# saltoricristiano/lidog

Hardware: AMD Instinct MI355X
Metric: LiDAR scans/sec, MinkUNet34+BEV training step @120k pts (higher is better)
Workload: dtype f32

## Files before the change

### include/lidog_amd.h

```cpp
#ifndef LIDOG_AMD_H
#define LIDOG_AMD_H

#include <stdint.h>

#ifdef __cplusplus
extern "C" {
#endif

const char *lidog_last_error(void);
int lidog_abi_version(void);


int64_t lidog_hash_capacity(int64_t n);

int lidog_coords_insert(const int32_t *coords, int64_t n, uint64_t *keys, int32_t *vals, int64_t cap,
                        int32_t *first_row, int64_t *n_unique_dev, int32_t *err_flag, void *stream);
int lidog_coords_insert_info(const int32_t *coords, int64_t n, uint64_t *keys, int32_t *vals, int64_t cap,
                             int32_t *first_row, int64_t *info, int32_t *err_flag, void *stream);

int lidog_coords_compact(const int32_t *first_row, int64_t n, const uint64_t *keys, int32_t *vals, int64_t cap,
                         const int32_t *coords, int32_t *unique_rows, int32_t *inverse, int32_t *scan_ws,
                         void *stream);

int lidog_coords_stride(const int32_t *coords_in, int64_t n_in, int32_t new_stride, uint64_t *keys,
// ... 121 lines not shown
                       const int32_t *pixel, int64_t n, int32_t C, int32_t B, int32_t H, int32_t W, int32_t pk,
                       int32_t ps, int32_t pp, int32_t Ho, int32_t Wo, float *gfeats , void *stream);

int lidog_conv2d_fwd(const float *x, const float *w, const float *bias, int32_t B, int32_t Cin, int32_t H,
                     int32_t W, int32_t Cout, int32_t ksize, int32_t stride, int32_t pad, float *y, void *stream);
int lidog_conv2d_dgrad(const float *gy, const float *w, int32_t B, int32_t Cin, int32_t H, int32_t W,
                       int32_t Cout, int32_t ksize, int32_t stride, int32_t pad, float *gx, float *ws,
                       void *stream);
int lidog_conv2d_wgrad(const float *x, const float *gy, int32_t B, int32_t Cin, int32_t H, int32_t W,
                       int32_t Cout, int32_t ksize, int32_t stride, int32_t pad, float *gw, float *gbias,
                       float *ws, int64_t ws_floats, void *stream);

int64_t lidog_conv2d_support_ws(int32_t B, int32_t Cin, int32_t H, int32_t W);
int lidog_conv2d_support(const int32_t *support, int32_t B, int32_t Cin, int32_t H, int32_t W, int32_t *act,
                         void *stream);
int lidog_conv2d_fwd_sparse(const float *x, const float *w, const int32_t *act, int32_t B, int32_t Cin, int32_t H,
                            int32_t W, int32_t Cout, float *y, float *ws, void *stream);
int lidog_conv2d_dgrad_sparse(const float *gy, const float *w, const int32_t *act, int32_t B, int32_t Cin, int32_t H,
                              int32_t W, int32_t Cout, float *gx, float *ws, void *stream);
int lidog_conv2d_support_work(const int32_t *act, int32_t B, int32_t Cin, int32_t H, int32_t W, int32_t Cout,
                              double *out, void *stream);
int64_t lidog_conv2d_wgrad_sparse_ws(int32_t B, int32_t Cin, int32_t H, int32_t W, int32_t Cout);
int lidog_conv2d_wgrad_sparse(const float *x, const float *gy, const int32_t *act, int32_t B, int32_t Cin, int32_t H,
                              int32_t W, int32_t Cout, float *gw, float *ws, int64_t ws_floats, void *stream);

int64_t lidog_dice_ws(int32_t C);
int lidog_dice_fwd(const float *logits, const int64_t *target, int64_t n, int32_t C, int64_t ignore_label,
                   int32_t has_ignore, float eps, int32_t soft, int32_t powerize, int32_t use_tmask, float offset,
                   double *ws, float *loss, float *coef, void *stream);
int lidog_dice_bwd(const float *logits, const int64_t *target, int64_t n, int32_t C, int64_t ignore_label,
// ... 243 lines not shown
```

### lidog_amd/_lib.py

```python
import ctypes
import os

import torch

_HERE = os.path.dirname(os.path.abspath(__file__))
SO_PATH = os.environ.get("LIDOG_SO") or os.path.join(_HERE, "_C", "liblidog_amd.so")

_i32, _i64, _p, _f, _d = ctypes.c_int32, ctypes.c_int64, ctypes.c_void_p, ctypes.c_float, ctypes.c_double

SIGNATURES = {
    "lidog_abi_version": [],
    "lidog_hash_capacity": [_i64],
    "lidog_coords_insert": [_p, _i64, _p, _p, _i64, _p, _p, _p, _p],
    "lidog_coords_insert_info": [_p, _i64, _p, _p, _i64, _p, _p, _p, _p],
    "lidog_coords_compact": [_p, _i64, _p, _p, _i64, _p, _p, _p, _p, _p],
    "lidog_coords_stride": [_p, _i64, _i32, _p, _p, _i64, _p, _p, _p, _p, _p, _p],
    "lidog_kernel_map": [_p, _i64, _p, _p, _i64, _p, _i32, _p, _p],
    "lidog_bitmap_words": [_i32, _i32, _i32, _i32, _i64],
    "lidog_bitmap_set": [_p, _i64, _i32, _i32, _i32, _i32, _i32, _i32, _i32, _i32, _p, _p, _p],
    "lidog_kernel_map_bits": [_p, _i64, _p, _p, _i64, _p, _i32, _p, _i32, _i32, _i32, _i32, _i32, _i32, _i32, _i32, _p, _p],
    "lidog_kernel_map_pairs": [_p, _i64, _i64, _i32, _p, _p, _p, _p, _p, _p, _p],
    "lidog_sconv_gemm_units": [_i32, _i32],
    "lidog_sconv_gemm": [_p, _p, _p, _p, _p, _p, _p, _i32, _i32, _i32, _p, _p, _i64, _p],
    "lidog_sconv_gemm_addend": [_p, _p, _p, _p, _p, _p, _i32, _i32, _i32, _p, _p, _p, _p],
# ... 46 lines not shown
    "lidog_colsum_ws": [_i32],
    "lidog_bn_eval_invstd": [_p, _f, _i32, _p, _p],
    "lidog_cat2": [_p, _i32, _p, _i32, _i64, _p, _p],
    "lidog_split2": [_p, _i32, _i32, _i64, _p, _p, _p],
    "lidog_relu_fwd": [_p, _i64, _p, _p],
    "lidog_relu_bwd": [_p, _p, _i64, _p, _p],
    "lidog_add": [_p, _p, _i64, _p, _p],
    "lidog_bev_winner": [_p, _i64, _p, _p, _i32, _i32, _i32, _i32, _p, _p, _p],
    "lidog_bev_pool_fwd": [_p, _i32, _p, _p, _i64, _i32, _i32, _i32, _i32, _i32, _i32, _i32, _i32, _p, _p, _p, _p],
    "lidog_bev_pool_bwd": [_p, _p, _p, _p, _i64, _i32, _i32, _i32, _i32, _i32, _i32, _i32, _i32, _i32, _p, _p],
    "lidog_conv2d_fwd": [_p, _p, _p, _i32, _i32, _i32, _i32, _i32, _i32, _i32, _i32, _p, _p],
    "lidog_conv2d_dgrad": [_p, _p, _i32, _i32, _i32, _i32, _i32, _i32, _i32, _i32, _p, _p, _p],
    "lidog_conv2d_wgrad": [_p, _p, _i32, _i32, _i32, _i32, _i32, _i32, _i32, _i32, _p, _p, _p, _i64, _p],
    "lidog_conv2d_support_ws": [_i32, _i32, _i32, _i32],
    "lidog_conv2d_support": [_p, _i32, _i32, _i32, _i32, _p, _p],
    "lidog_conv2d_fwd_sparse": [_p, _p, _p, _i32, _i32, _i32, _i32, _i32, _p, _p, _p],
    "lidog_conv2d_dgrad_sparse": [_p, _p, _p, _i32, _i32, _i32, _i32, _i32, _p, _p, _p],
    "lidog_conv2d_wgrad_sparse_ws": [_i32, _i32, _i32, _i32, _i32],
    "lidog_conv2d_wgrad_sparse": [_p, _p, _p, _i32, _i32, _i32, _i32, _i32, _p, _p, _i64, _p],
    "lidog_voxel_floor": [_p, _i64, _f, _f, _f, _i32, _p, _p],
    "lidog_label_vote": [_p, _p, _p, _i64, _i64, _i32, _p, _p],
    "lidog_bev_label_raster": [_p, _p, _i64, _p, _p, _p, _i32, _i32, _i32, _i32, _p, _p, _p, _p],
    "lidog_dice_ws": [_i32],
    "lidog_dice_fwd": [_p, _p, _i64, _i32, _i64, _i32, _f, _i32, _i32, _i32, _f, _p, _p, _p, _p],
    "lidog_dice_bwd": [_p, _p, _i64, _i32, _i64, _i32, _f, _i32, _i32, _p, _p, _p, _p],
    "lidog_dice_kitti_fwd": [_p, _p, _i64, _i32, _i64, _i32, _f, _i32, _i32, _f, _p, _p, _p, _p],
    "lidog_dice_kitti_bwd": [_p, _p, _i64, _i32, _i64, _i32, _f, _i32, _p, _p, _p, _p],
    "lidog_ce_ws": [_i32],
    "lidog_ce_fwd": [_p, _p, _i64, _i32, _i64, _i32, _p, _i32, _d, _d, _p, _p, _p, _p],
    "lidog_ce_bwd": [_p, _p, _i64, _i32, _i64, _i32, _p, _p, _p, _p, _p],
# ... 160 lines not shown
```

### lidog_amd/bev.py

```python
import os

import numpy as np
import torch
import torch.nn as nn

from . import me as ME
from ._lib import call, ptr

_LUTS = {}
SPARSE_CONV1 = os.environ.get("LIDOG_CONV1_SPARSE", "1") != "0"


def bev_image_size(bound, voxel=0.05):
    return int(np.float32((bound - (-bound)) / voxel))


def pixel_luts(bound, voxel=0.05):
    key = (float(bound), float(voxel))
    if key not in _LUTS:
        H = bev_image_size(bound, voxel)
        lo, hi = -int(H * 0.6), int(H * 0.6)
        c = np.arange(lo, hi, dtype=np.int32)
        v = c.astype(np.float32) * np.float32(voxel)
        inb = (np.float32(-bound) < v) & (v < np.float32(bound))
# ... 111 lines not shown
        return {"launches": len(self.records), "total_ms": ms, "executed_flops": flops}


HEAD_TIMER = None


def _timed(work):
    import contextlib
    t = HEAD_TIMER
    return HeadTimer._Span(t, work) if (t is not None and t.enabled) else contextlib.nullcontext()


class _Conv2dFn(torch.autograd.Function):

    @staticmethod
    def forward(ctx, x, w, bias, ksize, stride, pad, support):
        x, w = x.contiguous(), w.contiguous()
        B, Cin, H, W = x.shape
        Cout = w.shape[0]
        Ho, Wo = (H + 2 * pad - ksize) // stride + 1, (W + 2 * pad - ksize) // stride + 1
        y = torch.empty((B, Cout, Ho, Wo), dtype=torch.float32, device=x.device)
        act = None
        if support is not None and (ksize, stride, pad) == (3, 2, 1) and bias is None and Cin <= 128 \
                and Cout % 128 == 0:
            n_act = ME._lib.load().lidog_conv2d_support_ws(B, Cin, H, W)
            if tuple(support.shape) == tuple(x.shape):
                act = torch.empty(n_act, dtype=torch.int32, device=x.device)
                call("lidog_conv2d_support", ptr(support), B, Cin, H, W, ptr(act))
            elif support.dim() == 1 and support.numel() == n_act:
                act = support
                call("lidog_conv2d_support", None, B, Cin, H, W, ptr(act))
        dense = 2.0 * B * Ho * Wo * Cout * Cin * ksize * ksize
        if act is not None:
            ws = torch.empty(9 * Cin * Cout, dtype=torch.float32, device=x.device)
            with _timed((act, (B, Cin, H, W, Cout), 0)):
                call("lidog_conv2d_fwd_sparse", ptr(x), ptr(w), ptr(act), B, Cin, H, W, Cout, ptr(y), ptr(ws))
        elif ksize == 3:
            with _timed(dense):
                call("lidog_conv2d_fwd", ptr(x), ptr(w), ptr(bias), B, Cin, H, W, Cout, ksize, stride, pad, ptr(y))
        else:
            call("lidog_conv2d_fwd", ptr(x), ptr(w), ptr(bias), B, Cin, H, W, Cout, ksize, stride, pad, ptr(y))
        ctx.save_for_backward(x, w, act)
        ctx.cfg = (ksize, stride, pad, bias is not None)
        ctx.params = (w, bias)
        return y

    @staticmethod
    def backward(ctx, gy):
        x, w, act = ctx.saved_tensors
        ksize, stride, pad, has_bias = ctx.cfg
        gy = gy.contiguous()
        B, Cin, H, W = x.shape
        Cout = w.shape[0]
        gx = gw = gb = None
        lane_on = ME._WgradLane.active()
        behind = lane_on and ME._WgradLane.mode == 2

        def queue_wgrad():
            gw = ME._grad_out(ctx.params[0], w.shape)
            gb = ME._grad_out(ctx.params[1], (Cout,)) if has_bias else None
            if act is not None:
                n_ws = ME._lib.load().lidog_conv2d_wgrad_sparse_ws(B, Cin, H, W, Cout)
            else:
                n_ws = 32 * w.numel() if ksize == 3 else 4 * B * (w.numel() + Cout)

            def wgrad(gw, gb):
                ws = torch.empty(max(n_ws, 1), dtype=torch.float32, device=x.device)
                if act is not None:
                    with _timed((act, (B, Cin, H, W, Cout), 2)):
# ... 19 lines not shown
        if ctx.needs_input_grad[1] and not behind:
            gw, gb = queue_wgrad()
        if ctx.needs_input_grad[0]:
            gx = torch.empty_like(x)
            ws = torch.empty(9 * Cin * Cout, dtype=torch.float32, device=x.device) if ksize == 3 else None
            if act is not None:
                with _timed((act, (B, Cin, H, W, Cout), 1)):
                    call("lidog_conv2d_dgrad_sparse", ptr(gy), ptr(w), ptr(act), B, Cin, H, W, Cout, ptr(gx), ptr(ws))
            elif ksize == 3:
                with _timed(2.0 * gy.shape[0] * gy.shape[2] * gy.shape[3] * Cout * Cin * 9):
                    call("lidog_conv2d_dgrad", ptr(gy), ptr(w), B, Cin, H, W, Cout, ksize, stride, pad, ptr(gx), ptr(ws))
            else:
                call("lidog_conv2d_dgrad", ptr(gy), ptr(w), B, Cin, H, W, Cout, ksize, stride, pad, ptr(gx), ptr(ws))
        if ctx.needs_input_grad[1] and gw is None:
            gw, gb = queue_wgrad()
        return gx, gw, gb, None, None, None, None


def conv2d(x, conv, support=None):
    k, s, p = conv.kernel_size[0], conv.stride[0], conv.padding[0]
    return _Conv2dFn.apply(x, conv.weight, conv.bias, k, s, p, support)


class Encoder2D(nn.Module):

    def __init__(self, input_size, n_classes=7, binary_seg=False):
        super().__init__()
        if binary_seg:
            raise NotImplementedError("binary_seg is off in every LiDOG config")
        dbl = nn.Module()
        dbl.double_conv = nn.Sequential(
            nn.Conv2d(input_size, 256, kernel_size=3, padding=1, stride=2, bias=False), nn.BatchNorm2d(256),
            nn.ReLU(inplace=True),
            nn.Conv2d(256, 256, kernel_size=3, padding=1, stride=2, bias=False), nn.BatchNorm2d(256),
            nn.ReLU(inplace=True))
        down = nn.Module()
# ... 15 lines not shown
```

### lidog_amd/csrc/conv2d.hip

```cpp
#include "common.h"
#include "clock_stamp.h"

#include "conv2d.h"

#define WG_LD 129
__global__ __launch_bounds__(256) void k_conv_wgrad(IgParams p) {
    __shared__ float As[C2_KB * WG_LD];
    __shared__ float Bs[C2_KB * WG_LD];
    const int tid = threadIdx.x, lane = tid & 63, wave = tid >> 6;
    const int i0 = blockIdx.y * IG_T, j0 = blockIdx.x * IG_T;
    const int HoWo = p.Ho * p.Wo;
    const int k_begin = blockIdx.z * p.k_chunk;
    const int k_end = k_begin + p.k_chunk < p.Kd ? k_begin + p.k_chunk : p.Kd;
    const int kk = tid & 31, rg = tid >> 5;

    int cpk[16];
    unsigned a_mask = 0;
#pragma unroll
    for (int r = 0; r < 16; ++r) {
        int j = j0 + rg + 8 * r;
        cpk[r] = -1;
        int ci = j / 9;
        if (j < p.Nj) cpk[r] = wgrad_col(p, ci, j - ci * 9);
        a_mask |= (unsigned)(i0 + rg + 8 * r < p.Mi) << r;
// ... 164 lines not shown
void lidog_launch_repack_dgrad_all(const float *W, int Cin, int Cout, float *Wd, hipStream_t st) {
    const int64_t total = 9 * (int64_t)Cin * Cout;
    k_repack_dgrad_all<<<(unsigned)cdiv64(total, 256), 256, 0, st>>>(W, Cin, Cout, Wd);
}

__global__ __launch_bounds__(256) void k_sum_splits(const float *__restrict__ partial, int64_t n, int splits,
                                                    int64_t stride, float *__restrict__ out) {
    int64_t i = (int64_t)blockIdx.x * 256 + threadIdx.x;
    if (i >= n) return;
    float acc = partial[i];
    for (int s = 1; s < splits; ++s) acc += partial[(size_t)s * stride + i];
    out[i] = acc;
}

#define PW_MAXCO 8
__global__ __launch_bounds__(256) void k_pw_fwd(const float *__restrict__ X, const float *__restrict__ W,
                                                const float *__restrict__ bias, int Cin, int Cout, int64_t HW,
                                                int64_t total, float *__restrict__ Y) {
    int64_t e = (int64_t)blockIdx.x * 256 + threadIdx.x;
    if (e >= total) return;
    int64_t b = e / HW, pix = e - b * HW;
    float acc[PW_MAXCO];
#pragma unroll
    for (int co = 0; co < PW_MAXCO; ++co) acc[co] = 0.f;
    const float *x = X + (size_t)b * Cin * HW + pix;
    for (int ci = 0; ci < Cin; ++ci) {
        float v = x[(size_t)ci * HW];
#pragma unroll
        for (int co = 0; co < PW_MAXCO; ++co)
            if (co < Cout) acc[co] = __builtin_fmaf(v, W[co * Cin + ci], acc[co]);
    }
#pragma unroll
    for (int co = 0; co < PW_MAXCO; ++co)
        if (co < Cout) Y[((size_t)b * Cout + co) * HW + pix] = acc[co] + (bias ? bias[co] : 0.f);
}

__global__ __launch_bounds__(256) void k_pw_dgrad(const float *__restrict__ gY, const float *__restrict__ W, int Cin,
                                                  int Cout, int64_t HW, int64_t total, float *__restrict__ gX) {
    int64_t e = (int64_t)blockIdx.x * 256 + threadIdx.x;
    if (e >= total) return;
    int64_t b = e / HW, pix = e - b * HW;
    float g[PW_MAXCO];
#pragma unroll
    for (int co = 0; co < PW_MAXCO; ++co) g[co] = (co < Cout) ? gY[((size_t)b * Cout + co) * HW + pix] : 0.f;
    for (int ci = 0; ci < Cin; ++ci) {
        float acc = 0.f;
#pragma unroll
        for (int co = 0; co < PW_MAXCO; ++co)
            if (co < Cout) acc = __builtin_fmaf(g[co], W[co * Cin + ci], acc);
        gX[((size_t)b * Cin + ci) * HW + pix] = acc;
    }
}

#define PW_QUARTERS 4
__global__ __launch_bounds__(256) void k_pw_wgrad(const float *__restrict__ X, const float *__restrict__ gY, int Cin,
                                                  int Cout, int HW, float *__restrict__ partial) {
    __shared__ double red[2 * PW_MAXCO][4];
    const int ci = blockIdx.x, s = blockIdx.y;
    const int b = s / PW_QUARTERS, q = s % PW_QUARTERS;
    const int chunk = (HW + PW_QUARTERS - 1) / PW_QUARTERS;
    const int e0 = q * chunk, e1 = e0 + chunk < HW ? e0 + chunk : HW;
    const float *x = X + ((size_t)b * Cin + ci) * HW;
    const float *g = gY + (size_t)b * Cout * HW;
    double acc[PW_MAXCO], accb[PW_MAXCO];
#pragma unroll
    for (int co = 0; co < PW_MAXCO; ++co) { acc[co] = 0; accb[co] = 0; }
    for (int e = e0 + threadIdx.x; e < e1; e += 256) {
        float xv = x[e];
#pragma unroll
        for (int co = 0; co < PW_MAXCO; ++co)
            if (co < Cout) {
                float gv = g[(size_t)co * HW + e];
                acc[co] += (double)gv * (double)xv;
                accb[co] += (double)gv;
            }
    }
#pragma unroll
    for (int co = 0; co < PW_MAXCO; ++co) {
        double a = acc[co], bsum = accb[co];
#pragma unroll
        for (int d = 32; d >= 1; d >>= 1) { a += __shfl_down(a, d); bsum += __shfl_down(bsum, d); }
        if ((threadIdx.x & 63) == 0) { red[co][threadIdx.x >> 6] = a; red[PW_MAXCO + co][threadIdx.x >> 6] = bsum; }
    }
    __syncthreads();
    if (threadIdx.x < Cout) {
        int co = threadIdx.x;
        float *dst = partial + (size_t)s * (Cout * Cin + Cout);
        dst[co * Cin + ci] = (float)(red[co][0] + red[co][1] + red[co][2] + red[co][3]);
        if (ci == 0)
            dst[Cout * Cin + co] = (float)(red[PW_MAXCO + co][0] + red[PW_MAXCO + co][1] + red[PW_MAXCO + co][2] +
                                           red[PW_MAXCO + co][3]);
    }
}

void lidog_dgrad_classes(const float *gy, const float *Wd, int B, int Cin, int H, int W, int Cout, float *gx,
                         IgParams cls[4]) {
    const float *slab = Wd;
    for (int c = 0; c < 4; ++c) {
        IgParams &p = cls[c];
        p = IgParams{};
        p.Bm = gy; p.D = gx;
        p.Cin = Cin; p.H = H; p.W = W; p.Cout = Cout; p.Ho = c2_out_dim(H); p.Wo = c2_out_dim(W);
        p.py = c >> 1; p.px = c & 1;
        p.nky = p.py ? 2 : 1; p.ky0 = p.py ? 0 : 1;
        p.nkx = p.px ? 2 : 1; p.kx0 = p.px ? 0 : 1;
        p.Hc = (H - p.py + 1) / 2; p.Wc = (W - p.px + 1) / 2;
        const int nt = p.nky * p.nkx;
        p.Mi = Cin; p.Nj = B * p.Hc * p.Wc; p.Kd = Cout * nt;
        p.A = slab;
        slab += (int64_t)Cin * Cout * nt;
    }
}

extern "C" int lidog_conv2d_fwd(const float *x, const float *w, const float *bias, int32_t B, int32_t Cin, int32_t H,
                                int32_t W, int32_t Cout, int32_t ksize, int32_t stride, int32_t pad, float *y,
                                void *stream) {
    hipStream_t st = (hipStream_t)stream;
    if (ksize == 1) {
        LIDOG_REQUIRE(stride == 1 && pad == 0 && Cout <= PW_MAXCO, "conv2d_fwd: 1x1 path needs stride 1, Cout <= 8");
        int64_t HW = (int64_t)H * W, total = (int64_t)B * HW;
        if (total) k_pw_fwd<<<(unsigned)cdiv64(total, 256), 256, 0, st>>>(x, w, bias, Cin, Cout, HW, total, y);
        LIDOG_LAUNCH_CHECK();
        return 0;
    }
    LIDOG_REQUIRE(ksize == 3 && stride == 2 && pad == 1 && bias == nullptr,
                  "conv2d_fwd: MFMA path implements k3 s2 p1 without bias (Encoder2D)");
    LIDOG_REQUIRE((Cin * 9) % C2_KB == 0, "conv2d_fwd: Cin*9 must be a multiple of 32");
    IgParams p = {};
    p.A = w; p.Bm = x; p.D = y;
    p.Cin = Cin; p.H = H; p.W = W; p.Cout = Cout;
    p.Ho = c2_out_dim(H); p.Wo = c2_out_dim(W);
    p.Mi = Cout; p.Nj = B * p.Ho * p.Wo; p.Kd = Cin * 9;
    if (p.Nj == 0) return 0;
    LIDOG_REQUIRE((int64_t)B * Cin * H * W < ((int64_t)1 << 31) && (int64_t)p.Kd * 8 <= 24576,
                  "conv2d_fwd: tensor too large for 32-bit offsets / reduction table");
    IgClasses pc = {};
    pc.c[0] = p;
    pc.n = 1;
    pc.row_tiles[0] = (int)cdiv64(p.Mi, IG_T);
    pc.first[1] = (int)cdiv64(p.Nj, IG_T) * pc.row_tiles[0];
    k_conv_s2<IG_FWD, 2, 2, 2><<<(unsigned)pc.first[pc.n], 256, (size_t)p.Kd * sizeof(int2), st>>>(pc);
    LIDOG_LAUNCH_CHECK();
    return 0;
}

extern "C" int lidog_conv2d_dgrad(const float *gy, const float *w, int32_t B, int32_t Cin, int32_t H, int32_t W,
                                  int32_t Cout, int32_t ksize, int32_t stride, int32_t pad, float *gx, float *ws,
                                  void *stream) {
    hipStream_t st = (hipStream_t)stream;
    if (ksize == 1) {
        LIDOG_REQUIRE(stride == 1 && pad == 0 && Cout <= PW_MAXCO, "conv2d_dgrad: 1x1 path needs stride 1, Cout <= 8");
        int64_t HW = (int64_t)H * W, total = (int64_t)B * HW;
        if (total) k_pw_dgrad<<<(unsigned)cdiv64(total, 256), 256, 0, st>>>(gy, w, Cin, Cout, HW, total, gx);
        LIDOG_LAUNCH_CHECK();
        return 0;
    }
    LIDOG_REQUIRE(ksize == 3 && stride == 2 && pad == 1, "conv2d_dgrad: MFMA path implements k3 s2 p1");
    LIDOG_REQUIRE(ws != nullptr, "conv2d_dgrad: needs a 9*Cin*Cout float workspace for the repacked weights");
    LIDOG_REQUIRE(Cout % C2_KB == 0, "conv2d_dgrad: Cout must be a multiple of 32");
    LIDOG_REQUIRE((int64_t)B * Cout * c2_out_dim(H) * c2_out_dim(W) < ((int64_t)1 << 31) &&
                      (int64_t)Cout * 4 * 8 <= 24576,
                  "conv2d_dgrad: tensor too large for 32-bit offsets / reduction table");
    lidog_launch_repack_dgrad_all(w, Cin, Cout, ws, st);
    const bool rows96 = Cin % 128 != 0 && Cin % 96 == 0;
    IgClasses pc = {};
    IgParams cls_p[4];
    lidog_dgrad_classes(gy, ws, B, Cin, H, W, Cout, gx, cls_p);
    const int rt = rows96 ? Cin / 96 : (int)cdiv64(Cin, IG_T);
// ... 8 lines not shown
        if ((size_t)p.Kd * sizeof(int2) > tab) tab = (size_t)p.Kd * sizeof(int2);
    }
    if (pc.n > 0) {
        if (rows96) k_conv_s2<IG_DGRAD, 1, 3, 1><<<(unsigned)pc.first[pc.n], 256, tab, st>>>(pc);
        else k_conv_s2<IG_DGRAD, 2, 2, 2><<<(unsigned)pc.first[pc.n], 256, tab, st>>>(pc);
    }
    LIDOG_LAUNCH_CHECK();
    return 0;
}

extern "C" int lidog_conv2d_wgrad(const float *x, const float *gy, int32_t B, int32_t Cin, int32_t H, int32_t W,
                                  int32_t Cout, int32_t ksize, int32_t stride, int32_t pad, float *gw, float *gbias,
                                  float *ws, int64_t ws_floats, void *stream) {
    hipStream_t st = (hipStream_t)stream;
    if (ksize == 1) {
        LIDOG_REQUIRE(stride == 1 && pad == 0 && Cout <= PW_MAXCO, "conv2d_wgrad: 1x1 path needs stride 1, Cout <= 8");
        const int splits = B * PW_QUARTERS;
        const int64_t slab = (int64_t)Cout * Cin + Cout;
        LIDOG_REQUIRE(ws != nullptr && ws_floats >= splits * slab,
                      "conv2d_wgrad: 1x1 path needs a workspace of %lld floats", (long long)(splits * slab));
        LIDOG_REQUIRE((int64_t)H * W < ((int64_t)1 << 31), "conv2d_wgrad: image too large");
        if (B == 0 || H * W == 0) return 0;
        k_pw_wgrad<<<dim3((unsigned)Cin, (unsigned)splits), 256, 0, st>>>(x, gy, Cin, Cout, H * W, ws);
        k_sum_splits<<<(unsigned)cdiv64((int64_t)Cout * Cin, 256), 256, 0, st>>>(ws, (int64_t)Cout * Cin, splits, slab, gw);
        if (gbias) k_sum_splits<<<1, 256, 0, st>>>(ws + (int64_t)Cout * Cin, Cout, splits, slab, gbias);
        LIDOG_LAUNCH_CHECK();
        return 0;
    }
    LIDOG_REQUIRE(ksize == 3 && stride == 2 && pad == 1 && gbias == nullptr, "conv2d_wgrad: MFMA path implements k3 s2 p1");
    IgParams p = {};
    p.A = gy; p.Bm = x;
    p.Cin = Cin; p.H = H; p.W = W; p.Cout = Cout;
    p.Ho = c2_out_dim(H); p.Wo = c2_out_dim(W);
    p.Mi = Cout; p.Nj = Cin * 9; p.Kd = B * p.Ho * p.Wo;
    int64_t slab = (int64_t)p.Mi * p.Nj;
    int tiles = (int)(cdiv64(p.Nj, IG_T) * cdiv64(p.Mi, IG_T));
    int splits = 1024 / tiles;
    if (splits < 1) splits = 1;
// ... 18 lines not shown
```

### lidog_amd/csrc/conv2d_sparse.hip

```cpp
#include <vector>

#include "conv2d.h"

__global__ __launch_bounds__(256) void k_support_rowbits(const int32_t *__restrict__ sup, int64_t rows, int W,
                                                         int words, uint64_t *__restrict__ bits) {
    const int64_t row = (int64_t)blockIdx.x * 4 + (threadIdx.x >> 6);
    const int lane = threadIdx.x & 63;
    if (row >= rows) return;
    const int32_t *s = sup + row * W;
    for (int w = 0; w < words; ++w) {
        const int x = w * 64 + lane;
        const bool v = x < W && s[x] >= 0;
        const uint64_t bal = __ballot(v);
        if (lane == 0) bits[row * words + w] = bal;
    }
}

struct ListGeom {
    int C, H, W, Hc, Wc, Nj;
    int ya, ny, xlo, xhi;
    uint64_t mask;
};

__device__ __forceinline__ void tile_list(const uint64_t *__restrict__ bits, int words, const ListGeom &g,
// ... 108 lines not shown
    for (int cls = 0; cls < 4; ++cls) {
        int py = cls >> 1, px = cls & 1;
        int Hc = (H - py + 1) / 2, Wc = (W - px + 1) / 2;
        L.dgrad_tiles[cls] = (int)cdiv64((int64_t)B * Hc * Wc, IG_T);
        L.dgrad_off[cls] = off;
        off += (int64_t)L.dgrad_tiles[cls] * (C + 1);
    }
    L.total = off;
    return L;
}

extern "C" int64_t lidog_conv2d_support_ws(int32_t B, int32_t Cin, int32_t H, int32_t W) {
    return act_layout(B, Cin, H, W).total;
}

extern "C" int lidog_conv2d_support(const int32_t *support, int32_t B, int32_t Cin, int32_t H, int32_t W,
                                    int32_t *act, void *stream) {
    hipStream_t st = (hipStream_t)stream;
    LIDOG_REQUIRE(Cin >= 1 && Cin <= 128, "conv2d_support: 1 <= Cin <= 128");
    LIDOG_REQUIRE((int64_t)B * Cin * H * W < ((int64_t)1 << 31), "conv2d_support: tensor too large");
    if ((int64_t)B * H * W == 0) return 0;
    ActLayout L = act_layout(B, Cin, H, W);
    uint64_t *bits = reinterpret_cast<uint64_t *>(act + L.bits_off);
    int64_t rows = (int64_t)B * Cin * H;
    if (support)
        k_support_rowbits<<<(unsigned)cdiv64(rows, 4), 256, 0, st>>>(support, rows, W, L.words, bits);
    ListGeom g;
    g.C = Cin; g.H = H; g.W = W;
    g.Hc = c2_out_dim(H); g.Wc = c2_out_dim(W); g.Nj = B * g.Hc * g.Wc;
    g.ya = -1; g.ny = 3; g.xlo = -1; g.xhi = 1; g.mask = ~0ull;
    uint64_t *tbits = reinterpret_cast<uint64_t *>(act + L.tbits_off);
    k_tile_lists<<<(unsigned)L.fwd_tiles, 128, 0, st>>>(bits, L.words, g, act + L.fwd_off, tbits);
    k_group_lists<<<(unsigned)L.groups, 256, 0, st>>>(tbits, L.fwd_tiles, Cin, act + L.glists_off);
    ListGeom4 q;
    q.first[0] = 0;
    for (int cls = 0; cls < 4; ++cls) {
        int py = cls >> 1, px = cls & 1;
        g.Hc = (H - py + 1) / 2; g.Wc = (W - px + 1) / 2; g.Nj = B * g.Hc * g.Wc;
        g.ya = py; g.ny = 1; g.xlo = px; g.xhi = px;
        g.mask = px ? 0xAAAAAAAAAAAAAAAAull : 0x5555555555555555ull;
        q.g[cls] = g;
        q.off[cls] = L.dgrad_off[cls];
        q.first[cls + 1] = q.first[cls] + L.dgrad_tiles[cls];
    }
    if (q.first[4] > 0) k_tile_lists4<<<(unsigned)q.first[4], 128, 0, st>>>(bits, L.words, q, act);
    LIDOG_LAUNCH_CHECK();
    return 0;
}

__global__ __launch_bounds__(256) void k_conv_fwd_act(IgParams p, const int32_t *__restrict__ lists,
                                                      const float *__restrict__ Wt) {
    __shared__ __attribute__((aligned(16))) float As[C2_KB * IG_LD];
    __shared__ float Bs[C2_KB * IG_LD];
    extern __shared__ int2 s_tab[];
    const int tid = threadIdx.x, lane = tid & 63, wave = tid >> 6;
    const int i0 = blockIdx.y * IG_T, j0 = blockIdx.x * IG_T;
    const int HW = p.H * p.W, HoWo = p.Ho * p.Wo;
    const int kw = __builtin_amdgcn_readfirstlane(tid >> 7);
    const int32_t *lst = lists + (size_t)blockIdx.x * (p.Cin + 1);
    const int n_act = lst[0];
    const int Kd = n_act * 9, Kp = (Kd + C2_KB - 1) / C2_KB * C2_KB;

// ... 327 lines not shown
```

### lidog_amd/csrc/sconv.hip

```cpp
#include "common.h"
#include "stats_tail.h"
#include "sconv_mfma.h"

static int g_sparse_core = 1;
extern "C" int lidog_set_sparse_core(int32_t core) {
    LIDOG_REQUIRE(core == 0 || core == 1, "sparse core must be 0 (vector FMA) or 1 (MFMA f32)");
    g_sparse_core = core;
    return 0;
}
extern "C" int lidog_get_sparse_core(void) { return g_sparse_core; }

#define GM_TM 128
#define GM_BK 32
#define GM_SA 36

template <int CN>
__global__ __launch_bounds__(256) void k_sconv_gemm(const float *__restrict__ A, const int32_t *__restrict__ gather,
                                                    const float *__restrict__ B, const float *__restrict__ bias,
                                                    const int32_t *__restrict__ tile_k,
                                                    const int32_t *__restrict__ tile_row0,
                                                    const int32_t *__restrict__ tile_rows, int Cin, int Cout,
                                                    float *__restrict__ T, const int32_t *__restrict__ scatter) {
    constexpr int TN = 16 * CN;
    constexpr int BV = (GM_BK * TN / 4) / 256 > 0 ? (GM_BK * TN / 4) / 256 : 1;
// ... 708 lines not shown
#ifndef RED_STATS_ROWS
#define RED_STATS_ROWS 1
#endif
    int64_t nb = cdiv64(n, (int64_t)RB * RED_STATS_ROWS);
    if (nb > lidog_stats_max_blocks()) nb = lidog_stats_max_blocks();
    BnFinish fin = {eps, momentum, mean, invstd, running_mean, running_var, nullptr, nullptr};
    StatsTail tail;
    if (lidog_stats_tail_make(&tail, partial_ws, sums, count, C, fin, st)) return 1;
    k_sconv_reduce_rows4_stats<<<(unsigned)nb, 256, 0, st>>>((const float4 *)T, row_ptr, row_list, n, C4,
                                                             (const float4 *)bias, (float4 *)out, tail);
    lidog_stats_tail_finish(tail, (int)nb, st);
    LIDOG_LAUNCH_CHECK();
    return 0;
}

template <int C4>
__global__ __launch_bounds__(256) void k_sconv_cin1(const float *__restrict__ x, const int32_t *__restrict__ nbr,
                                                    const float4 *__restrict__ W, int64_t n, int K,
                                                    const float4 *__restrict__ bias, float4 *__restrict__ out) {
    extern __shared__ float4 s_w4[];
    for (int e = threadIdx.x; e < K * C4; e += 256) s_w4[e] = W[e];
    __syncthreads();
    const int64_t o = (int64_t)blockIdx.x * 256 + threadIdx.x;
    if (o >= n) return;
    float4 acc[C4];
#pragma unroll
    for (int c = 0; c < C4; ++c) acc[c] = make_float4(0.f, 0.f, 0.f, 0.f);
    int k = 0;
    for (; k + 5 <= K; k += 5) {
        int idx[5];
        float xv[5];
#pragma unroll
        for (int j = 0; j < 5; ++j) idx[j] = nbr[(int64_t)(k + j) * n + o];
#pragma unroll
        for (int j = 0; j < 5; ++j) xv[j] = x[idx[j] < 0 ? 0 : idx[j]];
#pragma unroll
        for (int j = 0; j < 5; ++j) {
            if (idx[j] < 0) continue;
#pragma unroll
            for (int c = 0; c < C4; ++c) {
                const float4 w = s_w4[(k + j) * C4 + c];
                acc[c].x += xv[j] * w.x;
                acc[c].y += xv[j] * w.y;
// ... 514 lines not shown
```

Baseline: 85.54.

## Overlap backward list building on side stream and specialise pointwise conv kernels

The sparse 2D conv support builder now launches the backward-only list kernels on the wgrad side stream, and skips them entirely when no gradient is needed. An event makes the backward pass wait for those lists. The 1x1 conv forward, dgrad and wgrad kernels are templated on Cout, stage weights in shared memory, batch channel loads, and block over input channels in dgrad and wgrad. The cin1 sparse conv adds a 25-wide unrolled gather loop for more loads in flight. These are several unrelated changes that trade register pressure and extra stream synchronisation for overlap and fewer redundant loads.

```diff
diff --git a/include/lidog_amd.h b/include/lidog_amd.h
--- a/include/lidog_amd.h
+++ b/include/lidog_amd.h
@@ -159,6 +159,8 @@
 int64_t lidog_conv2d_support_ws(int32_t B, int32_t Cin, int32_t H, int32_t W);
 int lidog_conv2d_support(const int32_t *support, int32_t B, int32_t Cin, int32_t H, int32_t W, int32_t *act,
                          void *stream);
+int lidog_conv2d_support_streams(const int32_t *support, int32_t B, int32_t Cin, int32_t H, int32_t W, int32_t *act,
+                                 int32_t backward_lists, void *side_stream, void *stream);
 int lidog_conv2d_fwd_sparse(const float *x, const float *w, const int32_t *act, int32_t B, int32_t Cin, int32_t H,
                             int32_t W, int32_t Cout, float *y, float *ws, void *stream);
 int lidog_conv2d_dgrad_sparse(const float *gy, const float *w, const int32_t *act, int32_t B, int32_t Cin, int32_t H,
diff --git a/lidog_amd/_lib.py b/lidog_amd/_lib.py
--- a/lidog_amd/_lib.py
+++ b/lidog_amd/_lib.py
@@ -84,6 +84,7 @@
     "lidog_conv2d_wgrad": [_p, _p, _i32, _i32, _i32, _i32, _i32, _i32, _i32, _i32, _p, _p, _p, _i64, _p],
     "lidog_conv2d_support_ws": [_i32, _i32, _i32, _i32],
     "lidog_conv2d_support": [_p, _i32, _i32, _i32, _i32, _p, _p],
+    "lidog_conv2d_support_streams": [_p, _i32, _i32, _i32, _i32, _p, _i32, _p, _p],
     "lidog_conv2d_fwd_sparse": [_p, _p, _p, _i32, _i32, _i32, _i32, _i32, _p, _p, _p],
     "lidog_conv2d_dgrad_sparse": [_p, _p, _p, _i32, _i32, _i32, _i32, _i32, _p, _p, _p],
     "lidog_conv2d_wgrad_sparse_ws": [_i32, _i32, _i32, _i32, _i32],
diff --git a/lidog_amd/bev.py b/lidog_amd/bev.py
--- a/lidog_amd/bev.py
+++ b/lidog_amd/bev.py
@@ -149,22 +149,32 @@
 class _Conv2dFn(torch.autograd.Function):
 
     @staticmethod
-    def forward(ctx, x, w, bias, ksize, stride, pad, support):
+    def forward(ctx, x, w, bias, ksize, stride, pad, support, grad_mode=True):
         x, w = x.contiguous(), w.contiguous()
         B, Cin, H, W = x.shape
         Cout = w.shape[0]
         Ho, Wo = (H + 2 * pad - ksize) // stride + 1, (W + 2 * pad - ksize) // stride + 1
         y = torch.empty((B, Cout, Ho, Wo), dtype=torch.float32, device=x.device)
         act = None
+        ctx.lists_ready = None
         if support is not None and (ksize, stride, pad) == (3, 2, 1) and bias is None and Cin <= 128 \
                 and Cout % 128 == 0:
             n_act = ME._lib.load().lidog_conv2d_support_ws(B, Cin, H, W)
+            src = None
             if tuple(support.shape) == tuple(x.shape):
                 act = torch.empty(n_act, dtype=torch.int32, device=x.device)
-                call("lidog_conv2d_support", ptr(support), B, Cin, H, W, ptr(act))
+                src = support
             elif support.dim() == 1 and support.numel() == n_act:
                 act = support
-                call("lidog_conv2d_support", None, B, Cin, H, W, ptr(act))
+            if act is not None:
+                backward = grad_mode and (ctx.needs_input_grad[0] or ctx.needs_input_grad[1])
+                lane = ME._WgradLane.get(x.device) if backward and ME._WgradLane.active() else None
+                call("lidog_conv2d_support_streams", ptr(src), B, Cin, H, W, ptr(act), int(backward),
+                     lane.raw if lane is not None else None)
+                if lane is not None:
+                    act.record_stream(lane.stream)
+                    ctx.lists_ready = torch.cuda.Event()
+                    ctx.lists_ready.record(lane.stream)
         dense = 2.0 * B * Ho * Wo * Cout * Cin * ksize * ksize
         if act is not None:
             ws = torch.empty(9 * Cin * Cout, dtype=torch.float32, device=x.device)
@@ -188,6 +198,8 @@
         B, Cin, H, W = x.shape
         Cout = w.shape[0]
         gx = gw = gb = None
+        if ctx.lists_ready is not None:
+            torch.cuda.current_stream(x.device).wait_event(ctx.lists_ready)
         lane_on = ME._WgradLane.active()
         behind = lane_on and ME._WgradLane.mode == 2
 
@@ -237,12 +249,12 @@
                 call("lidog_conv2d_dgrad", ptr(gy), ptr(w), B, Cin, H, W, Cout, ksize, stride, pad, ptr(gx), ptr(ws))
         if ctx.needs_input_grad[1] and gw is None:
             gw, gb = queue_wgrad()
-        return gx, gw, gb, None, None, None, None
+        return gx, gw, gb, None, None, None, None, None
 
 
 def conv2d(x, conv, support=None):
     k, s, p = conv.kernel_size[0], conv.stride[0], conv.padding[0]
-    return _Conv2dFn.apply(x, conv.weight, conv.bias, k, s, p, support)
+    return _Conv2dFn.apply(x, conv.weight, conv.bias, k, s, p, support, torch.is_grad_enabled())
 
 
 class Encoder2D(nn.Module):
diff --git a/lidog_amd/csrc/conv2d.hip b/lidog_amd/csrc/conv2d.hip
--- a/lidog_amd/csrc/conv2d.hip
+++ b/lidog_amd/csrc/conv2d.hip
@@ -202,84 +202,181 @@
 }
 
 #define PW_MAXCO 8
-__global__ __launch_bounds__(256) void k_pw_fwd(const float *__restrict__ X, const float *__restrict__ W,
-                                                const float *__restrict__ bias, int Cin, int Cout, int64_t HW,
-                                                int64_t total, float *__restrict__ Y) {
-    int64_t e = (int64_t)blockIdx.x * 256 + threadIdx.x;
+#define PW_CHUNK 256
+#define PW_BATCH 32
+#define PW_FWD_T 128
+template <int COUT>
+__global__ __launch_bounds__(PW_FWD_T) void k_pw_fwd(const float *__restrict__ X, const float *__restrict__ W,
+                                                     const float *__restrict__ bias, int Cin, int64_t HW,
+                                                     int64_t total, float *__restrict__ Y) {
+    __shared__ __attribute__((aligned(16))) float s_w[PW_CHUNK * PW_MAXCO];
+    const int64_t e = (int64_t)blockIdx.x * PW_FWD_T + threadIdx.x;
+    const bool live = e < total;
+    const int64_t ec = live ? e : total - 1;
+    const int64_t b = ec / HW, pix = ec - b * HW;
+    float acc[COUT];
+#pragma unroll
+    for (int co = 0; co < COUT; ++co) acc[co] = 0.f;
+    const float *x = X + (size_t)b * Cin * HW + pix;
+    for (int c0 = 0; c0 < Cin; c0 += PW_CHUNK) {
+        const int nc = Cin - c0 < PW_CHUNK ? Cin - c0 : PW_CHUNK;
+        if (c0) __syncthreads();
+        for (int i = threadIdx.x; i < nc * COUT; i += PW_FWD_T) {
+            const int ci = i / COUT, co = i - ci * COUT;
+            s_w[ci * PW_MAXCO + co] = W[co * Cin + c0 + ci];
+        }
+        __syncthreads();
+        int ci = 0;
+        for (; ci + PW_BATCH <= nc; ci += PW_BATCH) {
+            float v[PW_BATCH];
+#pragma unroll
+            for (int j = 0; j < PW_BATCH; ++j) v[j] = x[(size_t)(c0 + ci + j) * HW];
+#pragma unroll
+            for (int j = 0; j < PW_BATCH; ++j)
+#pragma unroll
+                for (int co = 0; co < COUT; ++co)
+                    acc[co] = __builtin_fmaf(v[j], s_w[(ci + j) * PW_MAXCO + co], acc[co]);
+        }
+        for (; ci < nc; ++ci) {
+            const float v = x[(size_t)(c0 + ci) * HW];
+#pragma unroll
+            for (int co = 0; co < COUT; ++co) acc[co] = __builtin_fmaf(v, s_w[ci * PW_MAXCO + co], acc[co]);
+        }
+    }
+    if (!live) return;
+#pragma unroll
+    for (int co = 0; co < COUT; ++co) Y[((size_t)b * COUT + co) * HW + pix] = acc[co] + (bias ? bias[co] : 0.f);
+}
+
+#define PW_DG_CI 32
+#define PW_DG_BATCH 8
+template <int COUT>
+__global__ __launch_bounds__(256) void k_pw_dgrad(const float *__restrict__ gY, const float *__restrict__ W, int Cin,
+                                                  int64_t HW, int64_t total, float *__restrict__ gX) {
+    __shared__ __attribute__((aligned(16))) float s_w[PW_DG_CI * PW_MAXCO];
+    const int c0 = blockIdx.y * PW_DG_CI;
+    const int nc = Cin - c0 < PW_DG_CI ? Cin - c0 : PW_DG_CI;
+    for (int i = threadIdx.x; i < nc * COUT; i += 256) {
+        const int ci = i / COUT, co = i - ci * COUT;
+        s_w[ci * PW_MAXCO + co] = W[co * Cin + c0 + ci];
+    }
+    __syncthreads();
+    const int64_t e = (int64_t)blockIdx.x * 256 + threadIdx.x;
     if (e >= total) return;
-    int64_t b = e / HW, pix = e - b * HW;
-    float acc[PW_MAXCO];
-#pragma unroll
-    for (int co = 0; co < PW_MAXCO; ++co) acc[co] = 0.f;
-    const float *x = X + (size_t)b * Cin * HW + pix;
-    for (int ci = 0; ci < Cin; ++ci) {
-        float v = x[(size_t)ci * HW];
-#pragma unroll
-        for (int co = 0; co < PW_MAXCO; ++co)
-            if (co < Cout) acc[co] = __builtin_fmaf(v, W[co * Cin + ci], acc[co]);
-    }
-#pragma unroll
-    for (int co = 0; co < PW_MAXCO; ++co)
-        if (co < Cout) Y[((size_t)b * Cout + co) * HW + pix] = acc[co] + (bias ? bias[co] : 0.f);
-}
-
-__global__ __launch_bounds__(256) void k_pw_dgrad(const float *__restrict__ gY, const float *__restrict__ W, int Cin,
-                                                  int Cout, int64_t HW, int64_t total, float *__restrict__ gX) {
-    int64_t e = (int64_t)blockIdx.x * 256 + threadIdx.x;
-    if (e >= total) return;
-    int64_t b = e / HW, pix = e - b * HW;
-    float g[PW_MAXCO];
-#pragma unroll
-    for (int co = 0; co < PW_MAXCO; ++co) g[co] = (co < Cout) ? gY[((size_t)b * Cout + co) * HW + pix] : 0.f;
-    for (int ci = 0; ci < Cin; ++ci) {
+    const int64_t b = e / HW, pix = e - b * HW;
+    float g[COUT];
+#pragma unroll
+    for (int co = 0; co < COUT; ++co) g[co] = gY[((size_t)b * COUT + co) * HW + pix];
+    float *gx = gX + ((size_t)b * Cin + c0) * HW + pix;
+    int ci = 0;
+    for (; ci + PW_DG_BATCH <= nc; ci += PW_DG_BATCH) {
+        float r[PW_DG_BATCH];
+#pragma unroll
+        for (int j = 0; j < PW_DG_BATCH; ++j) {
+            float acc = 0.f;
+#pragma unroll
+            for (int co = 0; co < COUT; ++co) acc = __builtin_fmaf(g[co], s_w[(ci + j) * PW_MAXCO + co], acc);
+            r[j] = acc;
+        }
+#pragma unroll
+        for (int j = 0; j < PW_DG_BATCH; ++j) gx[(size_t)(ci + j) * HW] = r[j];
+    }
+    for (; ci < nc; ++ci) {
         float acc = 0.f;
 #pragma unroll
-        for (int co = 0; co < PW_MAXCO; ++co)
-            if (co < Cout) acc = __builtin_fmaf(g[co], W[co * Cin + ci], acc);
-        gX[((size_t)b * Cin + ci) * HW + pix] = acc;
+        for (int co = 0; co < COUT; ++co) acc = __builtin_fmaf(g[co], s_w[ci * PW_MAXCO + co], acc);
+        gx[(size_t)ci * HW] = acc;
     }
 }
 
 #define PW_QUARTERS 4
+#define PW_WG_CB 4
+template <int COUT>
 __global__ __launch_bounds__(256) void k_pw_wgrad(const float *__restrict__ X, const float *__restrict__ gY, int Cin,
-                                                  int Cout, int HW, float *__restrict__ partial) {
-    __shared__ double red[2 * PW_MAXCO][4];
-    const int ci = blockIdx.x, s = blockIdx.y;
+                                                  int HW, float *__restrict__ partial) {
+    __shared__ double red[PW_WG_CB + 1][COUT][4];
+    const int ci0 = blockIdx.x * PW_WG_CB, s = blockIdx.y;
     const int b = s / PW_QUARTERS, q = s % PW_QUARTERS;
     const int chunk = (HW + PW_QUARTERS - 1) / PW_QUARTERS;
     const int e0 = q * chunk, e1 = e0 + chunk < HW ? e0 + chunk : HW;
-    const float *x = X + ((size_t)b * Cin + ci) * HW;
-    const float *g = gY + (size_t)b * Cout * HW;
-    double acc[PW_MAXCO], accb[PW_MAXCO];
-#pragma unroll
-    for (int co = 0; co < PW_MAXCO; ++co) { acc[co] = 0; accb[co] = 0; }
-    for (int e = e0 + threadIdx.x; e < e1; e += 256) {
-        float xv = x[e];
-#pragma unroll
-        for (int co = 0; co < PW_MAXCO; ++co)
-            if (co < Cout) {
-                float gv = g[(size_t)co * HW + e];
-                acc[co] += (double)gv * (double)xv;
-                accb[co] += (double)gv;
-            }
-    }
-#pragma unroll
-    for (int co = 0; co < PW_MAXCO; ++co) {
-        double a = acc[co], bsum = accb[co];
-#pragma unroll
-        for (int d = 32; d >= 1; d >>= 1) { a += __shfl_down(a, d); bsum += __shfl_down(bsum, d); }
-        if ((threadIdx.x & 63) == 0) { red[co][threadIdx.x >> 6] = a; red[PW_MAXCO + co][threadIdx.x >> 6] = bsum; }
+    const bool with_bias = ci0 == 0;
+    const float *x[PW_WG_CB];
+#pragma unroll
+    for (int c = 0; c < PW_WG_CB; ++c)
+        x[c] = X + ((size_t)b * Cin + (ci0 + c < Cin ? ci0 + c : Cin - 1)) * HW;
+    const float *g = gY + (size_t)b * COUT * HW;
+    double acc[PW_WG_CB][COUT], accb[COUT];
+#pragma unroll
+    for (int co = 0; co < COUT; ++co) {
+        accb[co] = 0;
+#pragma unroll
+        for (int c = 0; c < PW_WG_CB; ++c) acc[c][co] = 0;
+    }
+    int e = e0 + threadIdx.x;
+    for (; e + 256 < e1; e += 512) {
+        float xa[PW_WG_CB], xb[PW_WG_CB], ga[COUT], gb[COUT];
+#pragma unroll
+        for (int co = 0; co < COUT; ++co) { ga[co] = g[(size_t)co * HW + e]; gb[co] = g[(size_t)co * HW + e + 256]; }
+#pragma unroll
+        for (int c = 0; c < PW_WG_CB; ++c) { xa[c] = x[c][e]; xb[c] = x[c][e + 256]; }
+#pragma unroll
+        for (int co = 0; co < COUT; ++co) {
+#pragma unroll
+            for (int c = 0; c < PW_WG_CB; ++c) acc[c][co] += (double)ga[co] * (double)xa[c];
+            if (with_bias) accb[co] += (double)ga[co];
+        }
+#pragma unroll
+        for (int co = 0; co < COUT; ++co) {
+#pragma unroll
+            for (int c = 0; c < PW_WG_CB; ++c) acc[c][co] += (double)gb[co] * (double)xb[c];
+            if (with_bias) accb[co] += (double)gb[co];
+        }
+    }
+    if (e < e1) {
+#pragma unroll
+        for (int co = 0; co < COUT; ++co) {
+            const double gv = (double)g[(size_t)co * HW + e];
+#pragma unroll
+            for (int c = 0; c < PW_WG_CB; ++c) acc[c][co] += gv * (double)x[c][e];
+            if (with_bias) accb[co] += gv;
+        }
+    }
+    const int lane = threadIdx.x & 63, wv = threadIdx.x >> 6;
+#pragma unroll
+    for (int co = 0; co < COUT; ++co) {
+#pragma unroll
+        for (int c = 0; c < PW_WG_CB; ++c) {
+            double a = acc[c][co];
+#pragma unroll
+            for (int d = 32; d >= 1; d >>= 1) a += __shfl_down(a, d);
+            if (lane == 0) red[c][co][wv] = a;
+        }
+        if (with_bias) {
+            double a = accb[co];
+#pragma unroll
+            for (int d = 32; d >= 1; d >>= 1) a += __shfl_down(a, d);
+            if (lane == 0) red[PW_WG_CB][co][wv] = a;
+        }
     }
     __syncthreads();
-    if (threadIdx.x < Cout) {
-        int co = threadIdx.x;
-        float *dst = partial + (size_t)s * (Cout * Cin + Cout);
-        dst[co * Cin + ci] = (float)(red[co][0] + red[co][1] + red[co][2] + red[co][3]);
-        if (ci == 0)
-            dst[Cout * Cin + co] = (float)(red[PW_MAXCO + co][0] + red[PW_MAXCO + co][1] + red[PW_MAXCO + co][2] +
-                                           red[PW_MAXCO + co][3]);
-    }
-}
+    float *dst = partial + (size_t)s * (COUT * Cin + COUT);
+    const int t = threadIdx.x;
+    if (t < PW_WG_CB * COUT) {
+        const int c = t / COUT, co = t - c * COUT;
+        if (ci0 + c < Cin) dst[co * Cin + ci0 + c] = (float)(red[c][co][0] + red[c][co][1] + red[c][co][2] + red[c][co][3]);
+    } else if (with_bias && t < (PW_WG_CB + 1) * COUT) {
+        const int co = t - PW_WG_CB * COUT;
+        dst[COUT * Cin + co] = (float)(red[PW_WG_CB][co][0] + red[PW_WG_CB][co][1] + red[PW_WG_CB][co][2] +
+                                       red[PW_WG_CB][co][3]);
+    }
+}
+
+#define PW_SWITCH(cout, L)                                                                                           \
+    switch (cout) {                                                                                                   \
+        case 1: L(1); break; case 2: L(2); break; case 3: L(3); break; case 4: L(4); break;                          \
+        case 5: L(5); break; case 6: L(6); break; case 7: L(7); break; case 8: L(8); break;                          \
+        default: break;                                                                                               \
+    }
 
 void lidog_dgrad_classes(const float *gy, const float *Wd, int B, int Cin, int H, int W, int Cout, float *gx,
                          IgParams cls[4]) {
@@ -305,9 +402,12 @@
                                 void *stream) {
     hipStream_t st = (hipStream_t)stream;
     if (ksize == 1) {
-        LIDOG_REQUIRE(stride == 1 && pad == 0 && Cout <= PW_MAXCO, "conv2d_fwd: 1x1 path needs stride 1, Cout <= 8");
+        LIDOG_REQUIRE(stride == 1 && pad == 0 && Cout >= 1 && Cout <= PW_MAXCO,
+                      "conv2d_fwd: 1x1 path needs stride 1, Cout <= 8");
         int64_t HW = (int64_t)H * W, total = (int64_t)B * HW;
-        if (total) k_pw_fwd<<<(unsigned)cdiv64(total, 256), 256, 0, st>>>(x, w, bias, Cin, Cout, HW, total, y);
+#define PW_L(CO) k_pw_fwd<CO><<<(unsigned)cdiv64(total, PW_FWD_T), PW_FWD_T, 0, st>>>(x, w, bias, Cin, HW, total, y)
+        if (total) PW_SWITCH(Cout, PW_L)
+#undef PW_L
         LIDOG_LAUNCH_CHECK();
         return 0;
     }
@@ -337,9 +437,13 @@
                                   void *stream) {
     hipStream_t st = (hipStream_t)stream;
     if (ksize == 1) {
-        LIDOG_REQUIRE(stride == 1 && pad == 0 && Cout <= PW_MAXCO, "conv2d_dgrad: 1x1 path needs stride 1, Cout <= 8");
+        LIDOG_REQUIRE(stride == 1 && pad == 0 && Cout >= 1 && Cout <= PW_MAXCO,
+                      "conv2d_dgrad: 1x1 path needs stride 1, Cout <= 8");
         int64_t HW = (int64_t)H * W, total = (int64_t)B * HW;
-        if (total) k_pw_dgrad<<<(unsigned)cdiv64(total, 256), 256, 0, st>>>(gy, w, Cin, Cout, HW, total, gx);
+        const dim3 grid((unsigned)cdiv64(total, 256), (unsigned)cdiv64(Cin, PW_DG_CI));
+#define PW_L(CO) k_pw_dgrad<CO><<<grid, 256, 0, st>>>(gy, w, Cin, HW, total, gx)
+        if (total && Cin > 0) PW_SWITCH(Cout, PW_L)
+#undef PW_L
         LIDOG_LAUNCH_CHECK();
         return 0;
     }
@@ -378,14 +482,18 @@
                                   float *ws, int64_t ws_floats, void *stream) {
     hipStream_t st = (hipStream_t)stream;
     if (ksize == 1) {
-        LIDOG_REQUIRE(stride == 1 && pad == 0 && Cout <= PW_MAXCO, "conv2d_wgrad: 1x1 path needs stride 1, Cout <= 8");
+        LIDOG_REQUIRE(stride == 1 && pad == 0 && Cout >= 1 && Cout <= PW_MAXCO,
+                      "conv2d_wgrad: 1x1 path needs stride 1, Cout <= 8");
         const int splits = B * PW_QUARTERS;
         const int64_t slab = (int64_t)Cout * Cin + Cout;
         LIDOG_REQUIRE(ws != nullptr && ws_floats >= splits * slab,
                       "conv2d_wgrad: 1x1 path needs a workspace of %lld floats", (long long)(splits * slab));
         LIDOG_REQUIRE((int64_t)H * W < ((int64_t)1 << 31), "conv2d_wgrad: image too large");
         if (B == 0 || H * W == 0) return 0;
-        k_pw_wgrad<<<dim3((unsigned)Cin, (unsigned)splits), 256, 0, st>>>(x, gy, Cin, Cout, H * W, ws);
+        const dim3 grid((unsigned)cdiv64(Cin, PW_WG_CB), (unsigned)splits);
+#define PW_L(CO) k_pw_wgrad<CO><<<grid, 256, 0, st>>>(x, gy, Cin, H * W, ws)
+        PW_SWITCH(Cout, PW_L)
+#undef PW_L
         k_sum_splits<<<(unsigned)cdiv64((int64_t)Cout * Cin, 256), 256, 0, st>>>(ws, (int64_t)Cout * Cin, splits, slab, gw);
         if (gbias) k_sum_splits<<<1, 256, 0, st>>>(ws + (int64_t)Cout * Cin, Cout, splits, slab, gbias);
         LIDOG_LAUNCH_CHECK();
diff --git a/lidog_amd/csrc/conv2d_sparse.hip b/lidog_amd/csrc/conv2d_sparse.hip
--- a/lidog_amd/csrc/conv2d_sparse.hip
+++ b/lidog_amd/csrc/conv2d_sparse.hip
@@ -1,3 +1,4 @@
+#include <mutex>
 #include <vector>
 
 #include "conv2d.h"
@@ -146,12 +147,28 @@
     return act_layout(B, Cin, H, W).total;
 }
 
-extern "C" int lidog_conv2d_support(const int32_t *support, int32_t B, int32_t Cin, int32_t H, int32_t W,
-                                    int32_t *act, void *stream) {
+static int support_event(hipEvent_t *ev) {
+    static std::mutex mu;
+    static std::vector<hipEvent_t> pool;
+    int dev = 0;
+    LIDOG_CHECK_HIP(hipGetDevice(&dev));
+    std::lock_guard<std::mutex> lock(mu);
+    if (pool.size() < (size_t)dev + 1) pool.resize((size_t)dev + 1, nullptr);
+    if (!pool[dev]) LIDOG_CHECK_HIP(hipEventCreateWithFlags(&pool[dev], hipEventDisableTiming));
+    *ev = pool[dev];
+    return 0;
+}
+
+extern "C" int lidog_conv2d_support_streams(const int32_t *support, int32_t B, int32_t Cin, int32_t H, int32_t W,
+                                            int32_t *act, int32_t backward_lists, void *side_stream, void *stream) {
     hipStream_t st = (hipStream_t)stream;
     LIDOG_REQUIRE(Cin >= 1 && Cin <= 128, "conv2d_support: 1 <= Cin <= 128");
     LIDOG_REQUIRE((int64_t)B * Cin * H * W < ((int64_t)1 << 31), "conv2d_support: tensor too large");
     if ((int64_t)B * H * W == 0) return 0;
+    hipStream_t sb = (backward_lists && side_stream && side_stream != stream) ? (hipStream_t)side_stream : st;
+    hipEvent_t ev = nullptr;
+    if (sb != st)
+        if (int rc = support_event(&ev)) return rc;
     ActLayout L = act_layout(B, Cin, H, W);
     uint64_t *bits = reinterpret_cast<uint64_t *>(act + L.bits_off);
     int64_t rows = (int64_t)B * Cin * H;
@@ -163,7 +180,15 @@
     g.ya = -1; g.ny = 3; g.xlo = -1; g.xhi = 1; g.mask = ~0ull;
     uint64_t *tbits = reinterpret_cast<uint64_t *>(act + L.tbits_off);
     k_tile_lists<<<(unsigned)L.fwd_tiles, 128, 0, st>>>(bits, L.words, g, act + L.fwd_off, tbits);
-    k_group_lists<<<(unsigned)L.groups, 256, 0, st>>>(tbits, L.fwd_tiles, Cin, act + L.glists_off);
+    if (!backward_lists) {
+        LIDOG_LAUNCH_CHECK();
+        return 0;
+    }
+    if (sb != st) {
+        LIDOG_CHECK_HIP(hipEventRecord(ev, st));
+        LIDOG_CHECK_HIP(hipStreamWaitEvent(sb, ev, 0));
+    }
+    k_group_lists<<<(unsigned)L.groups, 256, 0, sb>>>(tbits, L.fwd_tiles, Cin, act + L.glists_off);
     ListGeom4 q;
     q.first[0] = 0;
     for (int cls = 0; cls < 4; ++cls) {
@@ -175,9 +200,14 @@
         q.off[cls] = L.dgrad_off[cls];
         q.first[cls + 1] = q.first[cls] + L.dgrad_tiles[cls];
     }
-    if (q.first[4] > 0) k_tile_lists4<<<(unsigned)q.first[4], 128, 0, st>>>(bits, L.words, q, act);
+    if (q.first[4] > 0) k_tile_lists4<<<(unsigned)q.first[4], 128, 0, sb>>>(bits, L.words, q, act);
     LIDOG_LAUNCH_CHECK();
     return 0;
+}
+
+extern "C" int lidog_conv2d_support(const int32_t *support, int32_t B, int32_t Cin, int32_t H, int32_t W,
+                                    int32_t *act, void *stream) {
+    return lidog_conv2d_support_streams(support, B, Cin, H, W, act, 1, nullptr, stream);
 }
 
 __global__ __launch_bounds__(256) void k_conv_fwd_act(IgParams p, const int32_t *__restrict__ lists,
diff --git a/lidog_amd/csrc/sconv.hip b/lidog_amd/csrc/sconv.hip
--- a/lidog_amd/csrc/sconv.hip
+++ b/lidog_amd/csrc/sconv.hip
@@ -746,6 +746,7 @@
     return 0;
 }
 
+#define SCONV_CIN1_PLANE 25
 template <int C4>
 __global__ __launch_bounds__(256) void k_sconv_cin1(const float *__restrict__ x, const int32_t *__restrict__ nbr,
                                                     const float4 *__restrict__ W, int64_t n, int K,
@@ -759,6 +760,26 @@
 #pragma unroll
     for (int c = 0; c < C4; ++c) acc[c] = make_float4(0.f, 0.f, 0.f, 0.f);
     int k = 0;
+    for (; k + SCONV_CIN1_PLANE <= K; k += SCONV_CIN1_PLANE) {
+        int idx[SCONV_CIN1_PLANE];
+        float xv[SCONV_CIN1_PLANE];
+#pragma unroll
+        for (int j = 0; j < SCONV_CIN1_PLANE; ++j) idx[j] = nbr[(int64_t)(k + j) * n + o];
+#pragma unroll
+        for (int j = 0; j < SCONV_CIN1_PLANE; ++j) xv[j] = x[idx[j] < 0 ? 0 : idx[j]];
+#pragma unroll
+        for (int j = 0; j < SCONV_CIN1_PLANE; ++j) {
+            if (idx[j] < 0) continue;
+#pragma unroll
+            for (int c = 0; c < C4; ++c) {
+                const float4 w = s_w4[(k + j) * C4 + c];
+                acc[c].x += xv[j] * w.x;
+                acc[c].y += xv[j] * w.y;
+                acc[c].z += xv[j] * w.z;
+                acc[c].w += xv[j] * w.w;
+            }
+        }
+    }
     for (; k + 5 <= K; k += 5) {
         int idx[5];
         float xv[5];
```

After: 86.26, median of 6. No clear change (+0.8%).
